# bramtoula/multi_robot_SLAM_separators

Measured on AMD Instinct MI355X. Metric: candidate keyframe-pair verifications/sec (NetVLAD NN + ORB match + RANSAC) @1/2/4/8 GPU, higher is better.
Workload: dtype u8+f16+f32+f64

## Files before the change

### multi_robot_slam_separators_amd/csrc/k_match.hip

```cpp
#include "sf_internal.hpp"
#include <type_traits>

namespace {

__device__ __forceinline__ uint32_t bcnt_acc(uint32_t x, uint32_t acc) {
  uint32_t r;
  asm("v_bcnt_u32_b32 %0, %1, %2" : "=v"(r) : "v"(x), "v"(acc));
  return r;
}

template <int W, int NQ>
__device__ __forceinline__ void knn2_scan(const uint32_t* __restrict__ dF, int Kf, const uint32_t (&q)[NQ][W],
                                          uint32_t (&k1)[NQ], uint32_t (&k2)[NQ]) {
#pragma unroll 4
  for (int f = 0; f < Kf; ++f) {
    const uint32_t* r = dF + (size_t)f * W;
    uint32_t x[W];
#pragma unroll
    for (int c = 0; c < W; ++c) x[c] = r[c];
#pragma unroll
    for (int j = 0; j < NQ; ++j) {
      uint32_t d = 0;
#pragma unroll
      for (int c = 0; c < W; ++c) d = bcnt_acc(x[c] ^ q[j][c], d);
      const uint32_t key = (d << 16) | (uint32_t)f;
      k2[j] = min(max(key, k1[j]), k2[j]);
      k1[j] = min(k1[j], key);
    }
  }
}

template <int W>
__device__ __forceinline__ void knn2_scan_l2(const uint32_t* __restrict__ dF, int Kf, const uint32_t (&q)[W], float& d1,
                                             float& d2, int& i1) {
#pragma unroll 1
  for (int f = 0; f < Kf; ++f) {
    const uint32_t* r = dF + (size_t)f * W;
    float s = 0.f;
#pragma unroll
    for (int c = 0; c < W; ++c) {
      const float d = __uint_as_float(q[c]) - __uint_as_float(r[c]);
      s = s + d * d;
    }
    if (s < d1) { d2 = d1; d1 = s; i1 = f; }
    else if (s < d2) { d2 = s; }
  }
}

template <int W>
__device__ __forceinline__ void knn2_scan_l2_halves(const uint32_t* __restrict__ dF, int Kf,
                                                    const uint32_t* __restrict__ qrow, float& d1, float& d2, int& i1) {
  static_assert(W == 128, "two halves of 64 dimensions");
  constexpr int H = 64, FB = 16;
#pragma unroll 1
  for (int f0 = 0; f0 < Kf; f0 += FB) {
    float s[FB];
#pragma unroll
    for (int j = 0; j < FB; ++j) s[j] = 0.f;
#pragma unroll 1
    for (int half = 0; half < 2; ++half) {
      uint32_t q[H];
      {
        const uint4* p = reinterpret_cast<const uint4*>(qrow + half * H);
#pragma unroll
        for (int c = 0; c < H / 4; ++c) {
          const uint4 v = p[c];
          q[4 * c] = v.x; q[4 * c + 1] = v.y; q[4 * c + 2] = v.z; q[4 * c + 3] = v.w;
        }
      }
#pragma unroll
      for (int j = 0; j < FB; ++j) {
        if (f0 + j < Kf) {
          const uint32_t* r = dF + (size_t)(f0 + j) * W + half * H;
          float a = s[j];
#pragma unroll
          for (int c = 0; c < H; ++c) {
            const float d = __uint_as_float(q[c]) - __uint_as_float(r[c]);
            a = a + d * d;
          }
          s[j] = a;
        }
      }
    }
#pragma unroll
    for (int j = 0; j < FB; ++j) {
      if (f0 + j < Kf) {
        if (s[j] < d1) { d2 = d1; d1 = s[j]; i1 = f0 + j; }
        else if (s[j] < d2) { d2 = s[j]; }
      }
    }
  }
}

template <int W>
__device__ __forceinline__ void load_desc(const uint32_t* __restrict__ base, int row, bool valid, uint32_t (&q)[W]) {
  const uint4* p = reinterpret_cast<const uint4*>(base + (size_t)(valid ? row : 0) * W);
#pragma unroll
  for (int c = 0; c < W / 4; ++c) {
    uint4 v = p[c];
    q[4 * c + 0] = v.x; q[4 * c + 1] = v.y; q[4 * c + 2] = v.z; q[4 * c + 3] = v.w;
  }
}

template <int W, int NQ, int NT, bool L2 = false>
__global__ void __launch_bounds__(NT)
k_match_global(StoreView st, const int32_t* __restrict__ pair_from, const int32_t* __restrict__ pair_to,
               float nndr, int min_inliers, int est, uint32_t* __restrict__ corr, CorrHeader* __restrict__ hdr,
               PassState* __restrict__ pass, int32_t* __restrict__ list, int32_t* __restrict__ counter) {
  extern __shared__ __attribute__((aligned(16))) int smem[];
  constexpr int NW = NT / 64;
  const int pair = blockIdx.x;
  const int tid = threadIdx.x;
  const int lane = tid & 63, wave = tid >> 6;
  const int kcap = st.kcap;
  const int sF = pair_from[pair], sT = pair_to[pair];
  if ((unsigned)sF >= (unsigned)st.n_slots || (unsigned)sT >= (unsigned)st.n_slots) {
    if (tid == 0) {
      CorrHeader h = {0, 0, 0, 0};
      hdr[pair] = h;
      PassState ps;
#pragma unroll
      for (int i = 0; i < 12; ++i) ps.T[i] = 0.f;
      ps.var = 1.0; ps.var_ang = 1.0; ps.is_null = 1; ps.inliers = 0; ps.matches = 0; ps.pad = 0;
      pass[pair] = ps;
    }
    return;
  }
  const int4 mF = st.meta[sF], mT = st.meta[sT];
  const int Kf = mF.x, Kt = mT.x;
  const uint32_t* dF = st.desc + (size_t)sF * kcap * W;
  const uint32_t* dT = st.desc + (size_t)sT * kcap * W;

  int* cnt = smem;
  int* owner = smem + kcap;
  int* misc = smem + 2 * kcap;

  for (int i = tid; i < Kf; i += NT) cnt[i] = 0;
  if (tid < 16) misc[tid] = 0;
  __syncthreads();

  int rejected = 0;
  if constexpr (L2) {
    static_assert(!L2 || NQ == 1, "one resident float row per lane");
    if (Kf > 0) {
      for (int base = 0; base < Kt; base += NT) {
        const int t = base + tid;
        float d1 = __int_as_float(0x7F800000), d2 = __int_as_float(0x7F800000);
        int i1 = -1;
        if constexpr (W > 64) {
          if (Kt - base - (tid & ~63) > 0)
            knn2_scan_l2_halves<W>(dF, Kf, dT + (size_t)(t < Kt ? t : 0) * W, d1, d2, i1);
        } else {
          uint32_t q[W];
          load_desc<W>(dT, t, t < Kt, q);
          if (Kt - base - (tid & ~63) > 0)
            knn2_scan_l2<W>(dF, Kf, q, d1, d2, i1);
        }
        if (t < Kt) {
          const bool acc = (Kf >= 2) && i1 >= 0 && !(d1 > nndr * d2);
          if (acc) {
            atomicAdd(&cnt[i1], 1);
            owner[i1] = t;
          } else {
            ++rejected;
          }
        }
      }
    }
  } else
  if (Kf > 0) {
    for (int base = 0; base < Kt; base += NQ * NT) {
      uint32_t q[NQ][W], k1[NQ], k2[NQ];
#pragma unroll
      for (int j = 0; j < NQ; ++j) {
        const int t = base + j * NT + tid;
        load_desc<W>(dT, t, t < Kt, q[j]);
        k1[j] = 0xFFFFFFFFu;
        k2[j] = 0xFFFFFFFFu;
      }
      const int wave_rows = Kt - base - (tid & ~63);
      const int groups = wave_rows <= 0 ? 0 : min(NQ, (wave_rows + NT - 1) / NT);
      if (groups == NQ) {
        knn2_scan<W, NQ>(dF, Kf, q, k1, k2);
      } else if (groups > 0) {
#pragma unroll
        for (int j = 0; j < NQ; ++j) {
          if (j < groups) {
            uint32_t qq[1][W], a1[1] = {0xFFFFFFFFu}, a2[1] = {0xFFFFFFFFu};
#pragma unroll
            for (int c = 0; c < W; ++c) qq[0][c] = q[j][c];
            knn2_scan<W, 1>(dF, Kf, qq, a1, a2);
            k1[j] = a1[0];
            k2[j] = a2[0];
          }
        }
      }
#pragma unroll
      for (int j = 0; j < NQ; ++j) {
        const int t = base + j * NT + tid;
        if (t < Kt) {
          const bool acc = (Kf >= 2) && !((float)(k1[j] >> 16) > nndr * (float)(k2[j] >> 16));
          if (acc) {
            const int f = (int)(k1[j] & 0xFFFFu);
            atomicAdd(&cnt[f], 1);
            owner[f] = t;
          } else {
            ++rejected;
          }
        }
      }
    }
  }
  for (int off = 32; off >= 1; off >>= 1) rejected += __shfl_xor(rejected, off);
  if (lane == 0 && rejected) atomicAdd(&misc[0], rejected);
  __syncthreads();

  uint32_t* out = corr + (size_t)pair * kcap;
  int running = 0;
  for (int base = 0; base < Kf; base += NT) {
    const int f = base + tid;
    const bool flag = (f < Kf) && (cnt[f] == 1);
    const unsigned long long bal = __ballot(flag);
    const int before = __popcll(bal & ((1ull << lane) - 1ull));
    if (lane == 0) misc[4 + wave] = __popcll(bal);
    __syncthreads();
    int woff = 0, total = 0;
#pragma unroll
    for (int w = 0; w < NW; ++w) {
      int c = misc[4 + w];
      if (w < wave) woff += c;
      total += c;
    }
    if (flag) out[running + woff + before] = (uint32_t)f | ((uint32_t)owner[f] << 16);
    running += total;
    __syncthreads();
  }
  const int n_corr = running;

  const int unique_to = (Kf > 0 && Kt > 0) ? misc[0] + n_corr : 0;
  const int words_from = (Kf > 0 && mF.y > 0) ? Kf : 0;
  const int words_to = (mT.y > 0) ? unique_to : 0;
  const bool motion = est == 0 ? (unique_to > 0 && words_from >= min_inliers && words_to >= min_inliers)
                    : est == 1 ? (unique_to > 0 && words_from >= min_inliers && unique_to >= min_inliers)
                               : (est == 3 && unique_to > 0 && ((words_from >= min_inliers && unique_to >= min_inliers) ||
                                                                (words_to >= min_inliers && Kf >= min_inliers)));
  const bool survivor = est == 3 ? (motion && n_corr > 0) : (motion && n_corr >= min_inliers && n_corr >= (est == 0 ? 3 : 4));
  if (motion && !survivor) {
    const float* xF = st.xyz + (size_t)sF * kcap * 3;
    const float* xT = st.xyz + (size_t)sT * kcap * 3;
    for (int i = tid; i < n_corr; i += NT) {
      uint32_t c = out[i];
      const float* a = xF + 3 * (c & 0xFFFFu);
      const float* b = xT + 3 * (c >> 16);
      bool ok = isfinite(a[0]) && isfinite(a[1]) && isfinite(a[2]);
      if (est == 0)
        ok = ok && isfinite(b[0]) && isfinite(b[1]) && isfinite(b[2]) && (a[0] != 0.f || a[1] != 0.f || a[2] != 0.f) &&
             (b[0] != 0.f || b[1] != 0.f || b[2] != 0.f);
      if (ok) atomicAdd(&misc[2], 1);
    }
    __syncthreads();
  }
  if (tid == 0) {
    CorrHeader h;
    h.n_corr = n_corr;
    h.words_from = words_from;
    h.words_to = words_to;
    h.words_to_2d = unique_to;
    hdr[pair] = h;
    PassState ps;
#pragma unroll
    for (int i = 0; i < 12; ++i) ps.T[i] = 0.f;
    ps.var = 1.0; ps.var_ang = 1.0;
    ps.is_null = 1;
    ps.inliers = 0;
    ps.matches = (motion && !survivor) ? misc[2] : 0;
    ps.pad = 0;
    pass[pair] = ps;
    if (survivor) {
      int pos = atomicAdd(counter, 1);
      list[pos] = pair;
    }
  }
}

__device__ __forceinline__ uint32_t min_u16(uint32_t a, uint32_t b) {
  uint32_t r;
  asm("v_min_u16 %0, %1, %2" : "=v"(r) : "v"(a), "v"(b));
  return r;
}
__device__ __forceinline__ uint32_t max_u16(uint32_t a, uint32_t b) {
  uint32_t r;
  asm("v_max_u16 %0, %1, %2" : "=v"(r) : "v"(a), "v"(b));
  return r;
}

constexpr int MATCH_CH = 16;

template <int W, int NQ>
__device__ __forceinline__ void knn2_step_lds(const uint32_t* fromD, int f, const uint32_t (&q)[NQ][W],
                                              uint32_t (&d1)[NQ], uint32_t (&d2)[NQ]) {
  const uint4* r = reinterpret_cast<const uint4*>(fromD + (size_t)f * W);
  uint32_t x[W];
#pragma unroll
  for (int c = 0; c < W / 4; ++c) {
    const uint4 v = r[c];
    x[4 * c] = v.x; x[4 * c + 1] = v.y; x[4 * c + 2] = v.z; x[4 * c + 3] = v.w;
  }
#pragma unroll
  for (int j = 0; j < NQ; ++j) {
    uint32_t d = 0;
#pragma unroll
    for (int c = 0; c < W; ++c) d = bcnt_acc(x[c] ^ q[j][c], d);
    d2[j] = min_u16(d2[j], max_u16(d, d1[j]));
    d1[j] = min_u16(d1[j], d);
  }
}

template <int W, int NQ>
__device__ __forceinline__ void knn2_scan_lds(const uint32_t* fromD, int Kf, const uint32_t (&q)[NQ][W],
                                              uint32_t (&d1)[NQ], uint32_t (&d2)[NQ], uint32_t (&chunk)[NQ]) {
  int c0 = 0;
  for (; c0 + MATCH_CH <= Kf; c0 += MATCH_CH) {
    uint32_t prev[NQ];
#pragma unroll
    for (int j = 0; j < NQ; ++j) prev[j] = d1[j];
#pragma unroll 4
    for (int u = 0; u < MATCH_CH; ++u) knn2_step_lds<W, NQ>(fromD, c0 + u, q, d1, d2);
#pragma unroll
    for (int j = 0; j < NQ; ++j) chunk[j] = ((d1[j] & 0xFFFFu) != (prev[j] & 0xFFFFu)) ? (uint32_t)c0 : chunk[j];
  }
  if (c0 < Kf) {
    uint32_t prev[NQ];
#pragma unroll
    for (int j = 0; j < NQ; ++j) prev[j] = d1[j];
    for (int f = c0; f < Kf; ++f) knn2_step_lds<W, NQ>(fromD, f, q, d1, d2);
#pragma unroll
    for (int j = 0; j < NQ; ++j) chunk[j] = ((d1[j] & 0xFFFFu) != (prev[j] & 0xFFFFu)) ? (uint32_t)c0 : chunk[j];
  }
}

typedef int mf_v8i __attribute__((ext_vector_type(8)));
typedef float mf_v16f __attribute__((ext_vector_type(16)));
constexpr float MF_FR = 1.f / 2048.f;
constexpr int MF_MAX_ROWS = 2048;

__device__ __forceinline__ mf_v8i fp4_spread_from(uint32_t x, uint32_t m88, uint32_t c22) {
  mf_v8i o = {0, 0, 0, 0, 0, 0, 0, 0};
  o[0] = (int)((x & m88) | c22);
  o[1] = (int)(x & 0x44444444u);
  o[2] = (int)(x & 0x22222222u);
  o[3] = (int)(x & 0x11111111u);
  return o;
}
__device__ __forceinline__ mf_v8i fp4_spread_to(uint32_t y, uint32_t m88, uint32_t c22) {
  mf_v8i o = {0, 0, 0, 0, 0, 0, 0, 0};
  const uint32_t n = ~y;
  o[0] = (int)((y & m88) | c22);
  o[1] = (int)(((n << 1) & m88) | c22);
  o[2] = (int)(((n << 2) & m88) | 0x44444444u);
  o[3] = (int)(((n << 3) & m88) | 0x66666666u);
  return o;
}

static inline size_t sf_match_lds_bytes(int kcap, int w) {
  const int behind = 2 * kcap + 16;
  return (size_t)(kcap * w + (behind > 32 * w ? behind : 32 * w)) * sizeof(int);
}

template <int KS>
__device__ __forceinline__ void load_raw(const uint32_t* p, uint32_t (&raw)[KS]) {
#pragma unroll
  for (int c = 0; c < KS / 4; ++c) {
    const uint4 v = reinterpret_cast<const uint4*>(p)[c];
    raw[4 * c] = v.x; raw[4 * c + 1] = v.y; raw[4 * c + 2] = v.z; raw[4 * c + 3] = v.w;
  }
}

__device__ __forceinline__ void top2_update16(const mf_v16f& v, float& b, float& s) {
  const float x0 = __builtin_amdgcn_fmed3f(b, v[0], v[1]);
  float ta, tb;
  asm("v_max3_f32 %0, %0, %4, %5\n\t"
      "v_med3_f32 %2, %0, %6, %7\n\t"
      "v_max3_f32 %0, %0, %6, %7\n\t"
      "v_max3_f32 %1, %1, %20, %2\n\t"
      "v_med3_f32 %2, %0, %8, %9\n\t"
      "v_max3_f32 %0, %0, %8, %9\n\t"
      "v_med3_f32 %3, %0, %10, %11\n\t"
      "v_max3_f32 %0, %0, %10, %11\n\t"
      "v_max3_f32 %1, %1, %2, %3\n\t"
      "v_med3_f32 %2, %0, %12, %13\n\t"
      "v_max3_f32 %0, %0, %12, %13\n\t"
      "v_med3_f32 %3, %0, %14, %15\n\t"
      "v_max3_f32 %0, %0, %14, %15\n\t"
      "v_max3_f32 %1, %1, %2, %3\n\t"
      "v_med3_f32 %2, %0, %16, %17\n\t"
      "v_max3_f32 %0, %0, %16, %17\n\t"
      "v_med3_f32 %3, %0, %18, %19\n\t"
      "v_max3_f32 %0, %0, %18, %19\n\t"
      "v_max3_f32 %1, %1, %2, %3"
      : "+v"(b), "+v"(s), "=&v"(ta), "=&v"(tb)
      : "v"(v[0]), "v"(v[1]), "v"(v[2]), "v"(v[3]), "v"(v[4]), "v"(v[5]), "v"(v[6]), "v"(v[7]), "v"(v[8]), "v"(v[9]),
        "v"(v[10]), "v"(v[11]), "v"(v[12]), "v"(v[13]), "v"(v[14]), "v"(v[15]), "v"(x0));
}

template <int W, int NTL, bool TAIL>
__device__ __forceinline__ void knn2_mfma_tile(const uint32_t* fromD, int Kf, int mt, int r, int h,
                                               const mf_v8i (&Bf)[NTL][W / 2], const float (&cin)[16],
                                               float (&b)[NTL], float (&s)[NTL], uint32_t m88, uint32_t c22,
                                               uint32_t (&raw)[W / 2], const uint32_t*& nxt) {
  constexpr int KS = W / 2;
  mf_v16f c0;
#pragma unroll
  for (int i = 0; i < 16; ++i) c0[i] = cin[i];
  if (TAIL) {
    const float lim = -(float)(Kf - mt * 32) * MF_FR;
#pragma unroll
    for (int i = 0; i < 16; ++i) c0[i] = c0[i] > lim ? c0[i] : -INFINITY;
  }
  mf_v8i Af[KS];
#pragma unroll
  for (int k = 0; k < KS; ++k) Af[k] = fp4_spread_from(raw[k], m88, c22);
  if (!TAIL) {
    nxt += 32 * W;
    load_raw<KS>(nxt, raw);
  }
#pragma unroll
  for (int j = 0; j < NTL; ++j) {
    b[j] += 32.f * MF_FR;
    s[j] += 32.f * MF_FR;
  }
#pragma unroll
  for (int j = 0; j < NTL; ++j) {
    mf_v16f acc = __builtin_amdgcn_mfma_scale_f32_32x32x64_f8f6f4(Af[0], Bf[j][0], c0, 4, 4, 0, 0, 0, 0);
#pragma unroll
    for (int k = 1; k < KS; ++k)
      acc = __builtin_amdgcn_mfma_scale_f32_32x32x64_f8f6f4(Af[k], Bf[j][k], acc, 4, 4, 0, 0, 0, 0);
    top2_update16(acc, b[j], s[j]);
  }
}

template <int W, int NTL>
struct MfB {
  mf_v8i Bf[NTL][W / 2];
  uint32_t psum;
};

template <int W, int NTL>
__device__ __forceinline__ void mf_load_b(const uint32_t* __restrict__ dT, int Kt, const int (&tile)[NTL], int lane,
                                          MfB<W, NTL>& B) {
  constexpr int KS = W / 2;
  const int r = lane & 31, h = lane >> 5;
  uint32_t m88, c22;
  asm volatile("v_mov_b32 %0, 0x88888888" : "=v"(m88));
  asm volatile("v_mov_b32 %0, 0x22222222" : "=v"(c22));
  uint32_t raw[NTL][KS];
#pragma unroll
  for (int j = 0; j < NTL; ++j) load_raw<KS>(dT + (size_t)min(tile[j] * 32 + r, Kt - 1) * W + KS * h, raw[j]);
  static_assert(NTL == 1 || 24 * W < 256, "a tile's popcount fits its byte");
  uint32_t pk = 0;
#pragma unroll
  for (int j = 0; j < NTL; ++j) {
    uint32_t p = 0;
#pragma unroll
    for (int k = 0; k < KS; ++k) {
      B.Bf[j][k] = fp4_spread_to(raw[j][k], m88, c22);
      p += __popc(raw[j][k] & 0x77777777u);
    }
    pk |= p << (8 * j);
  }
  B.psum = pk + __shfl_xor(pk, 32);
}

typedef int mf_v4i __attribute__((ext_vector_type(4)));

__device__ __forceinline__ void mf_pipe_half1(mf_v16f& acc, const mf_v4i& a0, const mf_v4i& a1, const mf_v4i& a2,
                                              const mf_v4i& a3, const mf_v4i& b0, const mf_v4i& b1, const mf_v16f& cin,
                                              const mf_v16f& old, float& b, float& s, float& x0, float& ta, float& tb) {
  asm volatile(
      "s_nop 1\n\t"
      "v_mfma_f32_32x32x64_f8f6f4 %[acc], %[a0], %[b0], %[cin] cbsz:4 blgp:4\n\t"
      "v_add_f32 %[b], 0x3c800000, %[b]\n\t"
      "v_add_f32 %[s], 0x3c800000, %[s]\n\t"
      "s_nop 1\n\t"
      "v_med3_f32 %[x0], %[b], %[o0], %[o1]\n\t"
      "v_max3_f32 %[b], %[b], %[o0], %[o1]\n\t"
      "v_mfma_f32_32x32x64_f8f6f4 %[acc], %[a1], %[b1], %[acc] cbsz:4 blgp:4\n\t"
      "v_med3_f32 %[ta], %[b], %[o2], %[o3]\n\t"
      "v_max3_f32 %[b], %[b], %[o2], %[o3]\n\t"
      "v_max3_f32 %[s], %[s], %[x0], %[ta]\n\t"
      "v_med3_f32 %[ta], %[b], %[o4], %[o5]\n\t"
      "v_max3_f32 %[b], %[b], %[o4], %[o5]\n\t"
      "v_med3_f32 %[tb], %[b], %[o6], %[o7]"
      : [acc] "=&v"(acc), [b] "+v"(b), [s] "+v"(s), [x0] "=&v"(x0), [ta] "=&v"(ta), [tb] "=&v"(tb)
      : [a0] "v"(a0), [a1] "v"(a1), "v"(a2), "v"(a3), [b0] "v"(b0), [b1] "v"(b1), [cin] "v"(cin), [o0] "v"(old[0]),
        [o1] "v"(old[1]), [o2] "v"(old[2]), [o3] "v"(old[3]), [o4] "v"(old[4]), [o5] "v"(old[5]), [o6] "v"(old[6]),
        [o7] "v"(old[7]));
}
__device__ __forceinline__ void mf_pipe_half2(mf_v16f& acc, const mf_v4i& a2, const mf_v4i& a3, const mf_v4i& b2,
                                              const mf_v4i& b3, const mf_v16f& old, float& b, float& s, float& ta,
                                              float& tb) {
  float x0;
  asm volatile(
      "v_mfma_f32_32x32x64_f8f6f4 %[acc], %[a2], %[b2], %[acc] cbsz:4 blgp:4\n\t"
      "v_max3_f32 %[b], %[b], %[o6], %[o7]\n\t"
      "v_max3_f32 %[s], %[s], %[ta], %[tb]\n\t"
      "v_med3_f32 %[x0], %[b], %[o8], %[o9]\n\t"
      "v_max3_f32 %[b], %[b], %[o8], %[o9]\n\t"
      "v_med3_f32 %[ta], %[b], %[o10], %[o11]\n\t"
      "v_max3_f32 %[b], %[b], %[o10], %[o11]\n\t"
      "v_mfma_f32_32x32x64_f8f6f4 %[acc], %[a3], %[b3], %[acc] cbsz:4 blgp:4\n\t"
      "v_max3_f32 %[s], %[s], %[x0], %[ta]\n\t"
      "v_med3_f32 %[ta], %[b], %[o12], %[o13]\n\t"
      "v_max3_f32 %[b], %[b], %[o12], %[o13]\n\t"
      "v_med3_f32 %[tb], %[b], %[o14], %[o15]\n\t"
      "v_max3_f32 %[b], %[b], %[o14], %[o15]\n\t"
      "v_max3_f32 %[s], %[s], %[ta], %[tb]"
      : [acc] "+v"(acc), [b] "+v"(b), [s] "+v"(s), [x0] "=&v"(x0), [ta] "+v"(ta), [tb] "+v"(tb)
      : [a2] "v"(a2), [a3] "v"(a3), [b2] "v"(b2), [b3] "v"(b3), [o6] "v"(old[6]), [o7] "v"(old[7]), [o8] "v"(old[8]),
        [o9] "v"(old[9]), [o10] "v"(old[10]), [o11] "v"(old[11]), [o12] "v"(old[12]), [o13] "v"(old[13]),
        [o14] "v"(old[14]), [o15] "v"(old[15]));
}
__device__ __forceinline__ void mf_pipe_drain(const mf_v16f& old, float& b, float& s) {
  float x0, ta, tb;
  asm volatile(
      "s_nop 11\n\t"
      "v_add_f32 %[b], 0x3c800000, %[b]\n\t"
      "v_add_f32 %[s], 0x3c800000, %[s]\n\t"
      "v_med3_f32 %[x0], %[b], %[o0], %[o1]\n\t"
      "v_max3_f32 %[b], %[b], %[o0], %[o1]\n\t"
      "v_med3_f32 %[ta], %[b], %[o2], %[o3]\n\t"
      "v_max3_f32 %[b], %[b], %[o2], %[o3]\n\t"
      "v_max3_f32 %[s], %[s], %[x0], %[ta]\n\t"
      "v_med3_f32 %[ta], %[b], %[o4], %[o5]\n\t"
      "v_max3_f32 %[b], %[b], %[o4], %[o5]\n\t"
      "v_med3_f32 %[tb], %[b], %[o6], %[o7]\n\t"
      "v_max3_f32 %[b], %[b], %[o6], %[o7]\n\t"
      "v_max3_f32 %[s], %[s], %[ta], %[tb]\n\t"
      "v_med3_f32 %[x0], %[b], %[o8], %[o9]\n\t"
      "v_max3_f32 %[b], %[b], %[o8], %[o9]\n\t"
      "v_med3_f32 %[ta], %[b], %[o10], %[o11]\n\t"
      "v_max3_f32 %[b], %[b], %[o10], %[o11]\n\t"
      "v_max3_f32 %[s], %[s], %[x0], %[ta]\n\t"
      "v_med3_f32 %[ta], %[b], %[o12], %[o13]\n\t"
      "v_max3_f32 %[b], %[b], %[o12], %[o13]\n\t"
      "v_med3_f32 %[tb], %[b], %[o14], %[o15]\n\t"
      "v_max3_f32 %[b], %[b], %[o14], %[o15]\n\t"
      "v_max3_f32 %[s], %[s], %[ta], %[tb]"
      : [b] "+v"(b), [s] "+v"(s), [x0] "=&v"(x0), [ta] "=&v"(ta), [tb] "=&v"(tb)
      : [o0] "v"(old[0]), [o1] "v"(old[1]), [o2] "v"(old[2]), [o3] "v"(old[3]), [o4] "v"(old[4]), [o5] "v"(old[5]),
        [o6] "v"(old[6]), [o7] "v"(old[7]), [o8] "v"(old[8]), [o9] "v"(old[9]), [o10] "v"(old[10]), [o11] "v"(old[11]),
        [o12] "v"(old[12]), [o13] "v"(old[13]), [o14] "v"(old[14]), [o15] "v"(old[15]));
}

template <int NTL>
__device__ __forceinline__ void mf_scan_tiles_pipe(const uint32_t* fromD, int n_full, int tail, const MfB<8, NTL>& B,
                                                   const float (&cin)[16], float (&b)[NTL], float (&s)[NTL],
                                                   uint32_t m88, uint32_t c22, uint32_t (&raw)[4],
                                                   const uint32_t*& nxt) {
  static_assert(NTL == 2 || NTL == 4, "tiles alternate between two accumulator tuples");
  mf_v4i B4[NTL][4];
#pragma unroll
  for (int j = 0; j < NTL; ++j) {
#pragma unroll
    for (int k = 0; k < 4; ++k) B4[j][k] = mf_v4i{B.Bf[j][k][0], B.Bf[j][k][1], B.Bf[j][k][2], B.Bf[j][k][3]};
  }
  mf_v16f c0, acc0, acc1;
#pragma unroll
  for (int i = 0; i < 16; ++i) { c0[i] = cin[i]; acc1[i] = -INFINITY; }
#pragma unroll 1
  for (int pass = 0; pass < 2; ++pass) {
    int n = n_full, step = 32 * 8;
    if (pass) {
      if (!tail) break;
      const float lim = -(float)tail * MF_FR;
#pragma unroll
      for (int i = 0; i < 16; ++i) c0[i] = c0[i] > lim ? c0[i] : -INFINITY;
      n = 1; step = 0;
    }
    for (int mt = 0; mt < n; ++mt) {
      mf_v4i A4[4];
#pragma unroll
      for (int k = 0; k < 4; ++k) {
        const mf_v8i a = fp4_spread_from(raw[k], m88, c22);
        A4[k] = mf_v4i{a[0], a[1], a[2], a[3]};
      }
      nxt += step;
      load_raw<4>(nxt, raw);
#pragma unroll
      for (int j = 0; j < NTL; j += 2) {
        constexpr int JP = NTL - 1;
        float x0, ta, tb;
        const int jp = j == 0 ? JP : j - 1;
        mf_pipe_half1(acc0, A4[0], A4[1], A4[2], A4[3], B4[j][0], B4[j][1], c0, acc1, b[jp], s[jp], x0, ta, tb);
        mf_pipe_half2(acc0, A4[2], A4[3], B4[j][2], B4[j][3], acc1, b[jp], s[jp], ta, tb);
        mf_pipe_half1(acc1, A4[0], A4[1], A4[2], A4[3], B4[j + 1][0], B4[j + 1][1], c0, acc0, b[j], s[j], x0, ta, tb);
        mf_pipe_half2(acc1, A4[2], A4[3], B4[j + 1][2], B4[j + 1][3], acc0, b[j], s[j], ta, tb);
      }
    }
  }
  mf_pipe_drain(acc1, b[NTL - 1], s[NTL - 1]);
}

__device__ __forceinline__ float mf_max(float a, float b) {
  float r;
  asm("v_max_f32 %0, %1, %2" : "=v"(r) : "v"(a), "v"(b));
  return r;
}
__device__ __forceinline__ float mf_min(float a, float b) {
  float r;
  asm("v_min_f32 %0, %1, %2" : "=v"(r) : "v"(a), "v"(b));
  return r;
}
__device__ __forceinline__ float mf_max3(float a, float b, float c) {
  float r;
  asm("v_max3_f32 %0, %1, %2, %3" : "=v"(r) : "v"(a), "v"(b), "v"(c));
  return r;
}

constexpr int mf_passes(int ntl) { return ntl == 1 ? 1 : ntl / 2; }

template <int W, int NTL, bool PIPE = false>
__device__ __forceinline__ void mf_scan(const uint32_t* fromD, int Kf, const MfB<W, NTL>& B, int lane,
                                        uint32_t (&d1)[mf_passes(NTL)], uint32_t (&d2)[mf_passes(NTL)],
                                        int (&idx)[mf_passes(NTL)]) {
  constexpr int KS = W / 2;
  const int r = lane & 31, h = lane >> 5;
  uint32_t m88, c22;
  asm volatile("v_mov_b32 %0, 0x88888888" : "=v"(m88));
  asm volatile("v_mov_b32 %0, 0x22222222" : "=v"(c22));
  float cin[16], b[NTL], s[NTL];
  const float hoff = h ? 4.f * MF_FR : 0.f;
#pragma unroll
  for (int i = 0; i < 16; ++i) cin[i] = -(float)((i & 3) + 8 * (i >> 2)) * MF_FR - hoff;
#pragma unroll
  for (int j = 0; j < NTL; ++j) { b[j] = -INFINITY; s[j] = -INFINITY; }
  const int n_full = Kf >> 5;
  uint32_t raw[KS];
  load_raw<KS>(fromD + (size_t)min(r, Kf - 1) * W + KS * h, raw);
  const uint32_t* nxt = fromD + (size_t)r * W + KS * h;
  if constexpr (PIPE && W == 8 && (NTL == 2 || NTL == 4)) {
    mf_scan_tiles_pipe<NTL>(fromD, n_full, Kf & 31, B, cin, b, s, m88, c22, raw, nxt);
  } else {
    for (int mt = 0; mt < n_full; ++mt) knn2_mfma_tile<W, NTL, false>(fromD, Kf, mt, r, h, B.Bf, cin, b, s, m88, c22, raw, nxt);
    if (Kf & 31) knn2_mfma_tile<W, NTL, true>(fromD, Kf, n_full, r, h, B.Bf, cin, b, s, m88, c22, raw, nxt);
  }
  const float org = (float)(32 * (((Kf + 31) >> 5) - 1)) * MF_FR;
#pragma unroll
  for (int p = 0; p < mf_passes(NTL); ++p) {
    float mb, ms, ob, os;
    int ts;
    if constexpr (NTL == 1) {
      mb = b[0]; ms = s[0]; ts = 24 * W - 2 * (int)B.psum;
      ob = __shfl_xor(mb, 32); os = __shfl_xor(ms, 32);
    } else {
      const int j0 = 2 * p, j1 = 2 * p + 1;
      mb = h ? b[j1] : b[j0]; ms = h ? s[j1] : s[j0]; ts = 24 * W - 2 * (int)((B.psum >> (16 * p + 8 * h)) & 0xFFu);
      ob = __shfl_xor(h ? b[j0] : b[j1], 32); os = __shfl_xor(h ? s[j0] : s[j1], 32);
    }
    const float nb = mf_max(mb, ob) - org;
    const float ns = mf_max3(mf_min(mb, ob), ms, os) - org;
    const float dot1 = 2.f * ceilf(nb * 0.5f), dot2 = 2.f * ceilf(ns * 0.5f);
    idx[p] = (int)((dot1 - nb) * 2048.f);
    d1[p] = (uint32_t)((32 * W - ts - (int)dot1) >> 1);
    d2[p] = ns == -INFINITY ? 0xFFFFu : (uint32_t)((32 * W - ts - (int)dot2) >> 1);
  }
}

template <int W, int NTL, bool PIPE = false>
__device__ __forceinline__ void knn2_mfma(const uint32_t* fromD, int Kf, const uint32_t* __restrict__ dT, int Kt,
                                          const int (&tile)[NTL], int lane, uint32_t (&d1)[mf_passes(NTL)],
                                          uint32_t (&d2)[mf_passes(NTL)], int (&idx)[mf_passes(NTL)]) {
  asm volatile("" : "+v"(lane));
  MfB<W, NTL> B;
  mf_load_b<W, NTL>(dT, Kt, tile, lane, B);
  mf_scan<W, NTL, PIPE>(fromD, Kf, B, lane, d1, d2, idx);
}

template <int W, int NQ, int NT, int MF_NTL = 2, bool MF_PIPE = false>
__device__ __forceinline__ bool match_v2_body(const StoreView& st, int pair, int sF, int sT, float nndr, int min_inliers,
                                              int est, uint32_t* out, CorrHeader& hdr_out, PassState& pass_out,
                                              int32_t* __restrict__ list, int32_t* __restrict__ counter, int* smem,
                                              unsigned long long* trace_row = nullptr) {
  constexpr int NW = NT / 64;
  const int tid = threadIdx.x;
  const int lane = tid & 63, wave = __builtin_amdgcn_readfirstlane(tid >> 6);
  const int kcap = st.kcap;
  if ((unsigned)sF >= (unsigned)st.n_slots || (unsigned)sT >= (unsigned)st.n_slots) {
    if (tid == 0) {
      CorrHeader h = {0, 0, 0, 0};
      hdr_out = h;
      PassState ps;
#pragma unroll
      for (int i = 0; i < 12; ++i) ps.T[i] = 0.f;
      ps.var = 1.0; ps.var_ang = 1.0; ps.is_null = 1; ps.inliers = 0; ps.matches = 0; ps.pad = 0;
      pass_out = ps;
    }
    return false;
  }
  const int4 mF = st.meta[sF], mT = st.meta[sT];
  const int Kf = mF.x, Kt = mT.x;
  const uint32_t* dF = st.desc + (size_t)sF * kcap * W;
  const uint32_t* dT = st.desc + (size_t)sT * kcap * W;

  uint32_t* fromD = reinterpret_cast<uint32_t*>(smem);
  int* cnt = smem + kcap * W;
  int* owner = cnt + kcap;
  int* misc = owner + kcap;

  {
    const uint4* src = reinterpret_cast<const uint4*>(dF);
    uint4* dst = reinterpret_cast<uint4*>(fromD);
    for (int i = tid; i < Kf * (W / 4); i += NT) dst[i] = src[i];
  }
  for (int i = tid; i < Kf; i += NT) cnt[i] = 0;
  if (tid < 16) misc[tid] = 0;
  __syncthreads();
  SF_TRACE_ROW_MARK(trace_row, 32);

  int rejected = 0;
  if constexpr (NQ == 0) {
    if (Kf > 0) {
      constexpr int NTL = W == 8 ? MF_NTL : 1;
      const int n_nt = (Kt + 31) >> 5;
      auto group = [&](auto g, int t0) {
        constexpr int G = decltype(g)::value, NP = mf_passes(G);
        int tl[G], f[NP];
        uint32_t a1[NP], a2[NP];
#pragma unroll
        for (int j = 0; j < G; ++j) tl[j] = t0 + j * NW;
        knn2_mfma<W, G, MF_PIPE>(fromD, Kf, dT, Kt, tl, lane, a1, a2, f);
#pragma unroll
        for (int p = 0; p < NP; ++p) {
          const int t = G == 1 ? tl[0] * 32 + lane : (tl[2 * p] + (lane >> 5) * NW) * 32 + (lane & 31);
          const bool on = (G > 1 || lane < 32) && t < Kt;
          const bool acc = (Kf >= 2) && !((float)a1[p] > nndr * (float)a2[p]);
          if (on && acc) {
            atomicAdd(&cnt[f[p]], 1);
            owner[f[p]] = t;
          }
          rejected += __popcll(__ballot(on && !acc));
        }
      };
      for (int t0 = wave; t0 < n_nt; t0 += NW * NTL) {
        const int avail = (n_nt - t0 + NW - 1) / NW;
        if constexpr (NTL >= 4) {
          if (avail >= 3) { group(std::integral_constant<int, 4>{}, t0); continue; }
        }
        if constexpr (NTL >= 2) {
          if (avail >= 2) { group(std::integral_constant<int, 2>{}, t0); continue; }
        }
        group(std::integral_constant<int, 1>{}, t0);
      }
    }
  } else if (Kf > 0) {
    for (int base = 0; base < Kt; base += NQ * NT) {

      uint32_t q[NQ][W], d1[NQ], d2[NQ], chunk[NQ];
#pragma unroll
      for (int j = 0; j < NQ; ++j) {
        const int t = base + j * NT + tid;
        load_desc<W>(dT, t, t < Kt, q[j]);
        d1[j] = 0xFFFFu;
        d2[j] = 0xFFFFu;
        chunk[j] = 0;
      }
      const int wave_rows = Kt - base - (tid & ~63);
      const int groups = wave_rows <= 0 ? 0 : min(NQ, (wave_rows + NT - 1) / NT);
      if (groups == NQ) {
        knn2_scan_lds<W, NQ>(fromD, Kf, q, d1, d2, chunk);
      } else if (groups > 0) {
#pragma unroll
        for (int j = 0; j < NQ; ++j) {
          if (j < groups) {
            uint32_t qq[1][W], a1[1] = {0xFFFFu}, a2[1] = {0xFFFFu}, ch[1] = {0};
#pragma unroll
            for (int c = 0; c < W; ++c) qq[0][c] = q[j][c];
            knn2_scan_lds<W, 1>(fromD, Kf, qq, a1, a2, ch);
            d1[j] = a1[0]; d2[j] = a2[0]; chunk[j] = ch[0];
          }
        }
      }
#pragma unroll
      for (int j = 0; j < NQ; ++j) {
        const int t = base + j * NT + tid;
        if (t < Kt) {
          const uint32_t b1 = d1[j] & 0xFFFFu, b2 = d2[j] & 0xFFFFu;
          const bool acc = (Kf >= 2) && !((float)b1 > nndr * (float)b2);
          if (acc) {
            int f = (int)chunk[j];
            const int fend = min(f + MATCH_CH, Kf);
            for (; f < fend; ++f) {
              const uint32_t* r = fromD + (size_t)f * W;
              uint32_t d = 0;
#pragma unroll
              for (int c = 0; c < W; ++c) d += __popc(r[c] ^ q[j][c]);
              if (d == b1) break;
            }
            atomicAdd(&cnt[f], 1);
            owner[f] = t;
          } else {
            ++rejected;
          }
        }
      }
    }
  }
  if constexpr (NQ != 0) {
    for (int off = 32; off >= 1; off >>= 1) rejected += __shfl_xor(rejected, off);
  }
  if (lane == 0 && rejected) atomicAdd(&misc[0], rejected);
  SF_TRACE_ROW_MARK(trace_row, 33);
  __syncthreads();
  SF_TRACE_ROW_MARK(trace_row, 34);

  int running = 0;
  for (int base = 0; base < Kf; base += NT) {
    const int f = base + tid;
    const bool flag = (f < Kf) && (cnt[f] == 1);
    const unsigned long long bal = __ballot(flag);
    const int before = __popcll(bal & ((1ull << lane) - 1ull));
    if (lane == 0) misc[4 + wave] = __popcll(bal);
    __syncthreads();
    int woff = 0, total = 0;
#pragma unroll
    for (int w = 0; w < NW; ++w) {
      int c = misc[4 + w];
      if (w < wave) woff += c;
      total += c;
    }
    if (flag) out[running + woff + before] = (uint32_t)f | ((uint32_t)owner[f] << 16);
    running += total;
    __syncthreads();
  }
  const int n_corr = running;
  SF_TRACE_ROW_MARK(trace_row, 35);

  const int unique_to = (Kf > 0 && Kt > 0) ? misc[0] + n_corr : 0;
  const int words_from = (Kf > 0 && mF.y > 0) ? Kf : 0;
  const int words_to = (mT.y > 0) ? unique_to : 0;
  const bool motion = est == 0 ? (unique_to > 0 && words_from >= min_inliers && words_to >= min_inliers)
                    : est == 1 ? (unique_to > 0 && words_from >= min_inliers && unique_to >= min_inliers)
                               : (est == 3 && unique_to > 0 && ((words_from >= min_inliers && unique_to >= min_inliers) ||
                                                                (words_to >= min_inliers && Kf >= min_inliers)));
  const bool survivor = est == 3 ? (motion && n_corr > 0) : (motion && n_corr >= min_inliers && n_corr >= (est == 0 ? 3 : 4));
  if (motion && !survivor) {
    const float* xF = st.xyz + (size_t)sF * kcap * 3;
    const float* xT = st.xyz + (size_t)sT * kcap * 3;
    for (int i = tid; i < n_corr; i += NT) {
      uint32_t c = out[i];
      const float* a = xF + 3 * (c & 0xFFFFu);
      const float* b = xT + 3 * (c >> 16);
      bool ok = isfinite(a[0]) && isfinite(a[1]) && isfinite(a[2]);
      if (est == 0)
        ok = ok && isfinite(b[0]) && isfinite(b[1]) && isfinite(b[2]) && (a[0] != 0.f || a[1] != 0.f || a[2] != 0.f) &&
             (b[0] != 0.f || b[1] != 0.f || b[2] != 0.f);
      if (ok) atomicAdd(&misc[2], 1);
    }
    __syncthreads();
  }
  if (tid == 0) {
    CorrHeader h;
    h.n_corr = n_corr;
    h.words_from = words_from;
    h.words_to = words_to;
    h.words_to_2d = unique_to;
    hdr_out = h;
    PassState ps;
#pragma unroll
    for (int i = 0; i < 12; ++i) ps.T[i] = 0.f;
    ps.var = 1.0; ps.var_ang = 1.0;
    ps.is_null = 1;
    ps.inliers = 0;
    ps.matches = (motion && !survivor) ? misc[2] : 0;
    ps.pad = 0;
    pass_out = ps;
    if (survivor && list) {
      int pos = atomicAdd(counter, 1);
      list[pos] = pair;
    }
  }
  return survivor;
}

template <int W, int NQ, int NT>
__global__ void __launch_bounds__(NT)
k_match_global_v2(StoreView st, const int32_t* __restrict__ pair_from, const int32_t* __restrict__ pair_to,
                  float nndr, int min_inliers, int est, uint32_t* __restrict__ corr, CorrHeader* __restrict__ hdr,
                  PassState* __restrict__ pass, int32_t* __restrict__ list, int32_t* __restrict__ counter) {
  extern __shared__ __attribute__((aligned(16))) int smem[];
  const int pair = (int)blockIdx.x;
  match_v2_body<W, NQ, NT>(st, pair, pair_from[pair], pair_to[pair], nndr, min_inliers, est, corr + (size_t)pair * st.kcap,
                           hdr[pair], pass[pair], list, counter, smem);
}

template <int W, int NT>
__global__ void __launch_bounds__(NT, 2)
k_match_global_mf(StoreView st, const int32_t* __restrict__ pair_from, const int32_t* __restrict__ pair_to,
                  float nndr, int min_inliers, int est, uint32_t* __restrict__ corr, CorrHeader* __restrict__ hdr,
                  PassState* __restrict__ pass, int32_t* __restrict__ list, int32_t* __restrict__ counter) {
  extern __shared__ __attribute__((aligned(16))) int smem[];
  const int pair = (int)blockIdx.x;
  match_v2_body<W, 0, NT, 4>(st, pair, pair_from[pair], pair_to[pair], nndr, min_inliers, est,
                             corr + (size_t)pair * st.kcap, hdr[pair], pass[pair], list, counter, smem);
}

template <int W, int NQ, int NT>
void launch_match_v2(sf_context* c, StoreView st, const int32_t* d_from, const int32_t* d_to, int n) {
  size_t lds = sf_match_lds_bytes(st.kcap, W);
  if (const char* v = getenv("SF_MATCH_LDS_PAD")) lds += (size_t)atoi(v);
  int32_t* counters = (int32_t*)c->w->counters.p;
  if constexpr (NQ == 0)
    hipLaunchKernelGGL((k_match_global_mf<W, NT>), dim3(n), dim3(NT), lds, c->stream, st, d_from, d_to,
                       c->dparams.nndr, c->dparams.min_inliers, sf_est_mode(c), (uint32_t*)c->w->corr1.p,
                       (CorrHeader*)c->w->hdr1.p, (PassState*)c->w->pass1.p, (int32_t*)c->w->list1.p, counters + 0);
  else
    hipLaunchKernelGGL((k_match_global_v2<W, NQ, NT>), dim3(n), dim3(NT), lds, c->stream, st, d_from, d_to,
                       c->dparams.nndr, c->dparams.min_inliers, sf_est_mode(c), (uint32_t*)c->w->corr1.p,
                       (CorrHeader*)c->w->hdr1.p, (PassState*)c->w->pass1.p, (int32_t*)c->w->list1.p, counters + 0);
}

template <int W, int NQ, int NT>
void launch_match(sf_context* c, StoreView st, const int32_t* d_from, const int32_t* d_to, int n) {
  const size_t lds = (size_t)(2 * st.kcap + 16) * sizeof(int);
  int32_t* counters = (int32_t*)c->w->counters.p;
  hipLaunchKernelGGL((k_match_global<W, NQ, NT>), dim3(n), dim3(NT), lds, c->stream, st, d_from, d_to,
                     c->dparams.nndr, c->dparams.min_inliers, sf_est_mode(c), (uint32_t*)c->w->corr1.p, (CorrHeader*)c->w->hdr1.p,
                     (PassState*)c->w->pass1.p, (int32_t*)c->w->list1.p, counters + 0);
}

template <int W>
void launch_match_l2(sf_context* c, StoreView st, const int32_t* d_from, const int32_t* d_to, int n) {
  const size_t lds = (size_t)(2 * st.kcap + 16) * sizeof(int);
  int32_t* counters = (int32_t*)c->w->counters.p;
  hipLaunchKernelGGL((k_match_global<W, 1, 256, true>), dim3(n), dim3(256), lds, c->stream, st, d_from, d_to,
                     c->dparams.nndr, c->dparams.min_inliers, sf_est_mode(c), (uint32_t*)c->w->corr1.p, (CorrHeader*)c->w->hdr1.p,
                     (PassState*)c->w->pass1.p, (int32_t*)c->w->list1.p, counters + 0);
}

}

int sf_launch_match_global(sf_context* c, StoreView st, const int32_t* d_from, const int32_t* d_to, int n) {
  if (n <= 0) return SF_OK;
  if (c->params.desc_type == 1) {
    sf_prof_begin(c, SF_K_MATCH);
    if (st.w == 64) launch_match_l2<64>(c, st, d_from, d_to, n);
    else launch_match_l2<128>(c, st, d_from, d_to, n);
    sf_prof_end(c, SF_K_MATCH);
    SF_HIP(c, hipGetLastError());
    return SF_OK;
  }
  int variant = c->match_variant;
  if (variant == 0) {
    const size_t lds_v2 = sf_match_lds_bytes(st.kcap, st.w);
    variant = lds_v2 <= 64 * 1024 ? (c->match_mfma && st.kcap <= MF_MAX_ROWS ? 10256 : 12256) : 2256;
  }
  sf_prof_begin(c, SF_K_MATCH);
#define SF_CASE(NQ_, NT_)                                                        \
  case NQ_ * 1000 + NT_:                                                         \
    if (st.w == 8) launch_match<8, NQ_, NT_>(c, st, d_from, d_to, n);            \
    else launch_match<16, NQ_, NT_>(c, st, d_from, d_to, n);                     \
    break;
  switch (variant) {
    SF_CASE(1, 256)
    SF_CASE(2, 256)
    SF_CASE(4, 128)
    SF_CASE(2, 128)
    SF_CASE(4, 256)
    SF_CASE(8, 64)
    SF_CASE(4, 64)
#define SF_CASE2(NQ_, NT_)                                                          \
  case 10000 + NQ_ * 1000 + NT_:                                                    \
    if (st.w == 8) launch_match_v2<8, NQ_, NT_>(c, st, d_from, d_to, n);            \
    else launch_match_v2<16, NQ_, NT_>(c, st, d_from, d_to, n);                     \
    break;
    SF_CASE2(0, 256)
    SF_CASE2(2, 256)
    SF_CASE2(1, 256)
    SF_CASE2(4, 128)
    SF_CASE2(2, 128)
#undef SF_CASE2
    default:
      sf_prof_end(c, SF_K_MATCH);
      return sf_fail(c, SF_EINVAL, "unknown match kernel variant %d", variant);
  }
#undef SF_CASE
  sf_prof_end(c, SF_K_MATCH);
  SF_HIP(c, hipGetLastError());
  return SF_OK;
}
```

Baseline: 23.59 million.

## Use approximate per-group top-2 in MFMA scan and repair second distance exactly

The MFMA top-2 reduction now takes a plain max over 15 of each 16-value group and runs a single med3/max3 against the last value, rather than a full med3/max3 chain across all 16. This cuts the VALU work interleaved with the MFMA instructions, but the second-best can be underestimated when both best values fall in the same group. To restore the ratio test, a new repair routine recomputes the exact Hamming second distance over the best match's 32-row tile (in 16-row slices) for candidates that pass the test or when nndr is negative. That adds divergent extra loads and popcount work proportional to the number of accepted matches, and its index-mask shortcut makes exact equivalence uncertain.

Result: faster. 24.39 million (median of 6 runs) (+3.4%).

```diff
diff --git a/multi_robot_slam_separators_amd/csrc/k_match.hip b/multi_robot_slam_separators_amd/csrc/k_match.hip
--- a/multi_robot_slam_separators_amd/csrc/k_match.hip
+++ b/multi_robot_slam_separators_amd/csrc/k_match.hip
@@ -377,30 +377,22 @@
 }
 
 __device__ __forceinline__ void top2_update16(const mf_v16f& v, float& b, float& s) {
-  const float x0 = __builtin_amdgcn_fmed3f(b, v[0], v[1]);
-  float ta, tb;
-  asm("v_max3_f32 %0, %0, %4, %5\n\t"
-      "v_med3_f32 %2, %0, %6, %7\n\t"
-      "v_max3_f32 %0, %0, %6, %7\n\t"
-      "v_max3_f32 %1, %1, %20, %2\n\t"
-      "v_med3_f32 %2, %0, %8, %9\n\t"
-      "v_max3_f32 %0, %0, %8, %9\n\t"
-      "v_med3_f32 %3, %0, %10, %11\n\t"
-      "v_max3_f32 %0, %0, %10, %11\n\t"
-      "v_max3_f32 %1, %1, %2, %3\n\t"
-      "v_med3_f32 %2, %0, %12, %13\n\t"
-      "v_max3_f32 %0, %0, %12, %13\n\t"
-      "v_med3_f32 %3, %0, %14, %15\n\t"
-      "v_max3_f32 %0, %0, %14, %15\n\t"
-      "v_max3_f32 %1, %1, %2, %3\n\t"
-      "v_med3_f32 %2, %0, %16, %17\n\t"
-      "v_max3_f32 %0, %0, %16, %17\n\t"
-      "v_med3_f32 %3, %0, %18, %19\n\t"
-      "v_max3_f32 %0, %0, %18, %19\n\t"
-      "v_max3_f32 %1, %1, %2, %3"
-      : "+v"(b), "+v"(s), "=&v"(ta), "=&v"(tb)
-      : "v"(v[0]), "v"(v[1]), "v"(v[2]), "v"(v[3]), "v"(v[4]), "v"(v[5]), "v"(v[6]), "v"(v[7]), "v"(v[8]), "v"(v[9]),
-        "v"(v[10]), "v"(v[11]), "v"(v[12]), "v"(v[13]), "v"(v[14]), "v"(v[15]), "v"(x0));
+  float t = __builtin_amdgcn_fmed3f(v[0], v[1], INFINITY);
+  float x;
+  asm("v_max3_f32 %[t], %[t], %[o2], %[o3]\n\t"
+      "v_max3_f32 %[t], %[t], %[o4], %[o5]\n\t"
+      "v_max3_f32 %[t], %[t], %[o6], %[o7]\n\t"
+      "v_max3_f32 %[t], %[t], %[o8], %[o9]\n\t"
+      "v_max3_f32 %[t], %[t], %[o10], %[o11]\n\t"
+      "v_max3_f32 %[t], %[t], %[o12], %[o13]\n\t"
+      "v_max_f32 %[t], %[t], %[o14]\n\t"
+      "v_med3_f32 %[x], %[b], %[t], %[o15]\n\t"
+      "v_max3_f32 %[b], %[b], %[t], %[o15]\n\t"
+      "v_max_f32 %[s], %[s], %[x]"
+      : [b] "+v"(b), [s] "+v"(s), [t] "+v"(t), [x] "=&v"(x)
+      : [o2] "v"(v[2]), [o3] "v"(v[3]), [o4] "v"(v[4]), [o5] "v"(v[5]), [o6] "v"(v[6]), [o7] "v"(v[7]), [o8] "v"(v[8]),
+        [o9] "v"(v[9]), [o10] "v"(v[10]), [o11] "v"(v[11]), [o12] "v"(v[12]), [o13] "v"(v[13]), [o14] "v"(v[14]),
+        [o15] "v"(v[15]));
 }
 
 template <int W, int NTL, bool TAIL>
@@ -475,78 +467,56 @@
 
 __device__ __forceinline__ void mf_pipe_half1(mf_v16f& acc, const mf_v4i& a0, const mf_v4i& a1, const mf_v4i& a2,
                                               const mf_v4i& a3, const mf_v4i& b0, const mf_v4i& b1, const mf_v16f& cin,
-                                              const mf_v16f& old, float& b, float& s, float& x0, float& ta, float& tb) {
+                                              const mf_v16f& old, float& b, float& s, float& t) {
   asm volatile(
       "s_nop 1\n\t"
       "v_mfma_f32_32x32x64_f8f6f4 %[acc], %[a0], %[b0], %[cin] cbsz:4 blgp:4\n\t"
       "v_add_f32 %[b], 0x3c800000, %[b]\n\t"
       "v_add_f32 %[s], 0x3c800000, %[s]\n\t"
-      "s_nop 1\n\t"
-      "v_med3_f32 %[x0], %[b], %[o0], %[o1]\n\t"
-      "v_max3_f32 %[b], %[b], %[o0], %[o1]\n\t"
+      "s_nop 4\n\t"
+      "v_max3_f32 %[t], %[o0], %[o1], %[o2]\n\t"
       "v_mfma_f32_32x32x64_f8f6f4 %[acc], %[a1], %[b1], %[acc] cbsz:4 blgp:4\n\t"
-      "v_med3_f32 %[ta], %[b], %[o2], %[o3]\n\t"
-      "v_max3_f32 %[b], %[b], %[o2], %[o3]\n\t"
-      "v_max3_f32 %[s], %[s], %[x0], %[ta]\n\t"
-      "v_med3_f32 %[ta], %[b], %[o4], %[o5]\n\t"
-      "v_max3_f32 %[b], %[b], %[o4], %[o5]\n\t"
-      "v_med3_f32 %[tb], %[b], %[o6], %[o7]"
-      : [acc] "=&v"(acc), [b] "+v"(b), [s] "+v"(s), [x0] "=&v"(x0), [ta] "=&v"(ta), [tb] "=&v"(tb)
+      "v_max3_f32 %[t], %[t], %[o3], %[o4]\n\t"
+      "v_max3_f32 %[t], %[t], %[o5], %[o6]\n\t"
+      "v_max3_f32 %[t], %[t], %[o7], %[o8]"
+      : [acc] "=&v"(acc), [b] "+v"(b), [s] "+v"(s), [t] "=&v"(t)
       : [a0] "v"(a0), [a1] "v"(a1), "v"(a2), "v"(a3), [b0] "v"(b0), [b1] "v"(b1), [cin] "v"(cin), [o0] "v"(old[0]),
         [o1] "v"(old[1]), [o2] "v"(old[2]), [o3] "v"(old[3]), [o4] "v"(old[4]), [o5] "v"(old[5]), [o6] "v"(old[6]),
-        [o7] "v"(old[7]));
+        [o7] "v"(old[7]), [o8] "v"(old[8]));
 }
 __device__ __forceinline__ void mf_pipe_half2(mf_v16f& acc, const mf_v4i& a2, const mf_v4i& a3, const mf_v4i& b2,
-                                              const mf_v4i& b3, const mf_v16f& old, float& b, float& s, float& ta,
-                                              float& tb) {
-  float x0;
+                                              const mf_v4i& b3, const mf_v16f& old, float& b, float& s, float& t) {
+  float x;
   asm volatile(
       "v_mfma_f32_32x32x64_f8f6f4 %[acc], %[a2], %[b2], %[acc] cbsz:4 blgp:4\n\t"
-      "v_max3_f32 %[b], %[b], %[o6], %[o7]\n\t"
-      "v_max3_f32 %[s], %[s], %[ta], %[tb]\n\t"
-      "v_med3_f32 %[x0], %[b], %[o8], %[o9]\n\t"
-      "v_max3_f32 %[b], %[b], %[o8], %[o9]\n\t"
-      "v_med3_f32 %[ta], %[b], %[o10], %[o11]\n\t"
-      "v_max3_f32 %[b], %[b], %[o10], %[o11]\n\t"
+      "v_max3_f32 %[t], %[t], %[o9], %[o10]\n\t"
+      "v_max3_f32 %[t], %[t], %[o11], %[o12]\n\t"
+      "v_max3_f32 %[t], %[t], %[o13], %[o14]\n\t"
       "v_mfma_f32_32x32x64_f8f6f4 %[acc], %[a3], %[b3], %[acc] cbsz:4 blgp:4\n\t"
-      "v_max3_f32 %[s], %[s], %[x0], %[ta]\n\t"
-      "v_med3_f32 %[ta], %[b], %[o12], %[o13]\n\t"
-      "v_max3_f32 %[b], %[b], %[o12], %[o13]\n\t"
-      "v_med3_f32 %[tb], %[b], %[o14], %[o15]\n\t"
-      "v_max3_f32 %[b], %[b], %[o14], %[o15]\n\t"
-      "v_max3_f32 %[s], %[s], %[ta], %[tb]"
-      : [acc] "+v"(acc), [b] "+v"(b), [s] "+v"(s), [x0] "=&v"(x0), [ta] "+v"(ta), [tb] "+v"(tb)
-      : [a2] "v"(a2), [a3] "v"(a3), [b2] "v"(b2), [b3] "v"(b3), [o6] "v"(old[6]), [o7] "v"(old[7]), [o8] "v"(old[8]),
-        [o9] "v"(old[9]), [o10] "v"(old[10]), [o11] "v"(old[11]), [o12] "v"(old[12]), [o13] "v"(old[13]),
-        [o14] "v"(old[14]), [o15] "v"(old[15]));
+      "v_med3_f32 %[x], %[b], %[t], %[o15]\n\t"
+      "v_max3_f32 %[b], %[b], %[t], %[o15]\n\t"
+      "v_max_f32 %[s], %[s], %[x]"
+      : [acc] "+v"(acc), [b] "+v"(b), [s] "+v"(s), [t] "+v"(t), [x] "=&v"(x)
+      : [a2] "v"(a2), [a3] "v"(a3), [b2] "v"(b2), [b3] "v"(b3), [o9] "v"(old[9]), [o10] "v"(old[10]), [o11] "v"(old[11]),
+        [o12] "v"(old[12]), [o13] "v"(old[13]), [o14] "v"(old[14]), [o15] "v"(old[15]));
 }
 __device__ __forceinline__ void mf_pipe_drain(const mf_v16f& old, float& b, float& s) {
-  float x0, ta, tb;
+  float t, x;
   asm volatile(
       "s_nop 11\n\t"
       "v_add_f32 %[b], 0x3c800000, %[b]\n\t"
       "v_add_f32 %[s], 0x3c800000, %[s]\n\t"
-      "v_med3_f32 %[x0], %[b], %[o0], %[o1]\n\t"
-      "v_max3_f32 %[b], %[b], %[o0], %[o1]\n\t"
-      "v_med3_f32 %[ta], %[b], %[o2], %[o3]\n\t"
-      "v_max3_f32 %[b], %[b], %[o2], %[o3]\n\t"
-      "v_max3_f32 %[s], %[s], %[x0], %[ta]\n\t"
-      "v_med3_f32 %[ta], %[b], %[o4], %[o5]\n\t"
-      "v_max3_f32 %[b], %[b], %[o4], %[o5]\n\t"
-      "v_med3_f32 %[tb], %[b], %[o6], %[o7]\n\t"
-      "v_max3_f32 %[b], %[b], %[o6], %[o7]\n\t"
-      "v_max3_f32 %[s], %[s], %[ta], %[tb]\n\t"
-      "v_med3_f32 %[x0], %[b], %[o8], %[o9]\n\t"
-      "v_max3_f32 %[b], %[b], %[o8], %[o9]\n\t"
-      "v_med3_f32 %[ta], %[b], %[o10], %[o11]\n\t"
-      "v_max3_f32 %[b], %[b], %[o10], %[o11]\n\t"
-      "v_max3_f32 %[s], %[s], %[x0], %[ta]\n\t"
-      "v_med3_f32 %[ta], %[b], %[o12], %[o13]\n\t"
-      "v_max3_f32 %[b], %[b], %[o12], %[o13]\n\t"
-      "v_med3_f32 %[tb], %[b], %[o14], %[o15]\n\t"
-      "v_max3_f32 %[b], %[b], %[o14], %[o15]\n\t"
-      "v_max3_f32 %[s], %[s], %[ta], %[tb]"
-      : [b] "+v"(b), [s] "+v"(s), [x0] "=&v"(x0), [ta] "=&v"(ta), [tb] "=&v"(tb)
+      "v_max3_f32 %[t], %[o0], %[o1], %[o2]\n\t"
+      "v_max3_f32 %[t], %[t], %[o3], %[o4]\n\t"
+      "v_max3_f32 %[t], %[t], %[o5], %[o6]\n\t"
+      "v_max3_f32 %[t], %[t], %[o7], %[o8]\n\t"
+      "v_max3_f32 %[t], %[t], %[o9], %[o10]\n\t"
+      "v_max3_f32 %[t], %[t], %[o11], %[o12]\n\t"
+      "v_max3_f32 %[t], %[t], %[o13], %[o14]\n\t"
+      "v_med3_f32 %[x], %[b], %[t], %[o15]\n\t"
+      "v_max3_f32 %[b], %[b], %[t], %[o15]\n\t"
+      "v_max_f32 %[s], %[s], %[x]"
+      : [b] "+v"(b), [s] "+v"(s), [t] "=&v"(t), [x] "=&v"(x)
       : [o0] "v"(old[0]), [o1] "v"(old[1]), [o2] "v"(old[2]), [o3] "v"(old[3]), [o4] "v"(old[4]), [o5] "v"(old[5]),
         [o6] "v"(old[6]), [o7] "v"(old[7]), [o8] "v"(old[8]), [o9] "v"(old[9]), [o10] "v"(old[10]), [o11] "v"(old[11]),
         [o12] "v"(old[12]), [o13] "v"(old[13]), [o14] "v"(old[14]), [o15] "v"(old[15]));
@@ -589,12 +559,12 @@
 #pragma unroll
       for (int j = 0; j < NTL; j += 2) {
         constexpr int JP = NTL - 1;
-        float x0, ta, tb;
+        float t;
         const int jp = j == 0 ? JP : j - 1;
-        mf_pipe_half1(acc0, A4[0], A4[1], A4[2], A4[3], B4[j][0], B4[j][1], c0, acc1, b[jp], s[jp], x0, ta, tb);
-        mf_pipe_half2(acc0, A4[2], A4[3], B4[j][2], B4[j][3], acc1, b[jp], s[jp], ta, tb);
-        mf_pipe_half1(acc1, A4[0], A4[1], A4[2], A4[3], B4[j + 1][0], B4[j + 1][1], c0, acc0, b[j], s[j], x0, ta, tb);
-        mf_pipe_half2(acc1, A4[2], A4[3], B4[j + 1][2], B4[j + 1][3], acc0, b[j], s[j], ta, tb);
+        mf_pipe_half1(acc0, A4[0], A4[1], A4[2], A4[3], B4[j][0], B4[j][1], c0, acc1, b[jp], s[jp], t);
+        mf_pipe_half2(acc0, A4[2], A4[3], B4[j][2], B4[j][3], acc1, b[jp], s[jp], t);
+        mf_pipe_half1(acc1, A4[0], A4[1], A4[2], A4[3], B4[j + 1][0], B4[j + 1][1], c0, acc0, b[j], s[j], t);
+        mf_pipe_half2(acc1, A4[2], A4[3], B4[j + 1][2], B4[j + 1][3], acc0, b[j], s[j], t);
       }
     }
   }
@@ -674,6 +644,30 @@
   MfB<W, NTL> B;
   mf_load_b<W, NTL>(dT, Kt, tile, lane, B);
   mf_scan<W, NTL, PIPE>(fromD, Kf, B, lane, d1, d2, idx);
+}
+
+template <int W>
+__device__ __forceinline__ uint32_t mf_repair_d2(const uint32_t* fromD, int Kf, const uint32_t* __restrict__ q_row, int idx,
+                                                 uint32_t d2) {
+  if ((idx & 27) == 27) return d2;
+  uint32_t q[W];
+  load_raw<W>(q_row, q);
+  const int base = (idx & ~31) + (idx & 4);
+#pragma unroll 1
+  for (int g = 0; g < 32; g += 8) {
+#pragma unroll
+    for (int k = 0; k < 4; ++k) {
+      const int row = base + g + k;
+      uint32_t x[W];
+      load_raw<W>(fromD + (size_t)row * W, x);
+      uint32_t d = 0;
+#pragma unroll
+      for (int c = 0; c < W; ++c) d = bcnt_acc(x[c] ^ q[c], d);
+      const bool other = row < Kf && row != idx && (g + k) != 27;
+      d2 = other ? min(d2, d) : d2;
+    }
+  }
+  return d2;
 }
 
 template <int W, int NQ, int NT, int MF_NTL = 2, bool MF_PIPE = false>
@@ -733,7 +727,14 @@
         for (int p = 0; p < NP; ++p) {
           const int t = G == 1 ? tl[0] * 32 + lane : (tl[2 * p] + (lane >> 5) * NW) * 32 + (lane & 31);
           const bool on = (G > 1 || lane < 32) && t < Kt;
-          const bool acc = (Kf >= 2) && !((float)a1[p] > nndr * (float)a2[p]);
+          bool acc = (Kf >= 2) && !((float)a1[p] > nndr * (float)a2[p]);
+          const bool redo = on && Kf >= 2 && (acc || nndr < 0.f);
+          if (__ballot(redo)) {
+            if (redo) {
+              a2[p] = mf_repair_d2<W>(fromD, Kf, dT + (size_t)t * W, f[p], a2[p]);
+              acc = !((float)a1[p] > nndr * (float)a2[p]);
+            }
+          }
           if (on && acc) {
             atomicAdd(&cnt[f[p]], 1);
             owner[f[p]] = t;
```
